# tomershay100/mp3-steganography-lib

Measured on AMD Instinct MI355X. Metric: MP3 frames/sec (decode+re-encode) @44.1kHz stereo 128kbps, 1→8 GPU, higher is better.
Workload: dtype f64 (decode) / int32 (encode); 1 GPU; 10000-frame full decode->stego-embed->re-encode pipeline per MI355X (BASELINE configs[2]); MP3 main data + side info resident in HBM, MP3 frames out; the message cursor chain is decided and the serial chains of the rate loop are checked on the device inside every step; frames_per_gpu=10000, channels=2, message_bits=536, chain_verdict_units_to_redo=0, message_variant_entries=1874, parallelism=frames sharded over 1 GPU(s), no collective

## Files before the change

mp3-steganography-lib_amd/csrc/k_pack.hpp:

```cpp
#pragma once

namespace mp3s {

constexpr int PACK_DW = 372;
constexpr int PACK_FAM = 260;
constexpr int PACK_PT_QUAD = 4 * PACK_FAM, PACK_PT_NONE = PACK_PT_QUAD + 32, PACK_PT = PACK_PT_NONE + 1;
#define MP3S_PS_OVERFLOW 1
#define MP3S_PS_BAD_TABLE 2

__device__ __forceinline__ void lds_put(uint32_t *fb, uint32_t pos, uint32_t val, int n)
{
    if (n <= 0) return;
    const uint32_t d = pos >> 5, o = pos & 31;
    const uint64_t w = (uint64_t)val << (64 - o - n);
    atomicOr(&fb[d], (uint32_t)(w >> 32));
    if ((uint32_t)w) atomicOr(&fb[d + 1], (uint32_t)w);
}

__device__ __forceinline__ int pack_wave_sum(int v, bool on) { return (int)wave_add_u32(on ? (uint32_t)v : 0u); }

__global__ __launch_bounds__(256) void k_enc_pack(
    const int16_t *__restrict__ ix, const mp3s_gr_out *__restrict__ gr, const int32_t *__restrict__ en, int n_frames,
    int sri, int bri, int whole_slots, const uint32_t *__restrict__ frame_off, const uint8_t *__restrict__ padding,
    uint8_t *__restrict__ mp3, int32_t *__restrict__ scfsi_out, int32_t *__restrict__ status, int32_t *__restrict__ sync,
    int f_begin )
{
    __shared__ uint32_t fb3[3][PACK_DW];
    __shared__ uint32_t pt[PACK_PT];
    __shared__ int wg_err;
    const int wave0 = __builtin_amdgcn_readfirstlane(threadIdx.x >> 6), lane0 = threadIdx.x & 63;
    for (int i = threadIdx.x; i < 1024; i += 256) {
        const uint32_t len = i < 256 ? c_tab.hlen13[i] : (i < 512 ? c_tab.hlen15[i - 256] : (i < 768 ? c_tab.hlen16[i - 512] : c_tab.hlen24[i - 768]));
        pt[(i >> 8) * PACK_FAM + (i & 255)] = (&c_tab.hcod[0][0])[i] | (len << 24);
    }
    if (threadIdx.x < 16) {
        pt[PACK_PT_QUAD + threadIdx.x] = (uint32_t)c_tab.hcod_c1a[threadIdx.x] | ((uint32_t)c_tab.hlen_c1a[threadIdx.x] << 24);
        pt[PACK_PT_QUAD + 16 + threadIdx.x] = (15u - threadIdx.x) | (4u << 24);
    }
    if (threadIdx.x == 0) pt[PACK_PT_NONE] = 0;
    for (int i = threadIdx.x; i < 3 * PACK_DW; i += 256) (&fb3[0][0])[i] = 0;
    if (threadIdx.x == 0) wg_err = 0;
    __syncthreads();
    int rot = 0;
    for (int f = f_begin + blockIdx.x; f < n_frames; f += gridDim.x) {
    const int lane = lane0, tid = (int)threadIdx.x;
    int lane_p = lane0, wave = wave0;
    asm volatile("" : "+v"(lane_p), "+s"(wave));
    uint32_t *fb = fb3[rot];
    {
        uint32_t *cl = fb3[rot == 2 ? 0 : rot + 1];
        for (int i = tid; i < PACK_DW; i += 256) cl[i] = 0;
    }
    const int pad = padding[f];
    int p23v[4];
    {
        const int bits_per_frame = 8 * (whole_slots + pad);
        const int mean_bits = (bits_per_frame - 288) / 2;
        int sum = 0;
#pragma unroll
        for (int e = 0; e < 4; e++) {
            p23v[e] = __builtin_amdgcn_readfirstlane(gr[((long)f * 2 + (e & 1)) * 2 + (e >> 1)].part2_3_length);
            sum += p23v[e];
        }
        int stuffing = 2 * mean_bits - sum + ((mean_bits & 1) ? 1 : 0);
        if (stuffing < 0) stuffing = 0;
        if (stuffing) {
            if (p23v[0] + stuffing < 4095) p23v[0] += stuffing;
            else
#pragma unroll
                for (int e = 0; e < 4; e++) {
                    const int extra = 4095 - p23v[e], now = extra < stuffing ? extra : stuffing;
                    p23v[e] += now; stuffing -= now;
                }
        }
    }
    const int e = wave, grn = e >> 1, ch = e & 1;
    const long u = ((long)f * 2 + ch) * 2 + grn;
    const mp3s_gr_out &g = gr[u];
    if (wave < 2) {
        const long u0 = ((long)f * 2 + wave) * 2, u1 = u0 + 1;
        int a = 0, tot21 = 0;
        if (lane_p < 22) {
            a = en[u0 * 22 + lane] - en[u1 * 22 + lane];
            a = a < 0 ? -a : a;
        }
        tot21 = __builtin_amdgcn_readlane(a, 21);
        int sc = lane_p < 21 ? a : 0;
        sc += __builtin_amdgcn_update_dpp(0, sc, 0x111, 0xf, 0xf, false);
        sc += __builtin_amdgcn_update_dpp(0, sc, 0x112, 0xf, 0xf, false);
        sc += __builtin_amdgcn_update_dpp(0, sc, 0x114, 0xf, 0xf, false);
        sc += __builtin_amdgcn_update_dpp(0, sc, 0x118, 0xf, 0xf, false);
        const int row0 = __builtin_amdgcn_readlane(sc, 15);
        const int p5 = __builtin_amdgcn_readlane(sc, 5), p10 = __builtin_amdgcn_readlane(sc, 10), q20 = __builtin_amdgcn_readlane(sc, 20);
        const int tp = row0 + q20;
        int cond = 2 + (gr[u0].xrmax != 0) + (gr[u1].xrmax != 0);
        if (tot21 < 10) cond++;
        if (tp < 100) cond++;
        const int band_sum[4] = {p5, p10 - p5, row0 - p10, q20};
        uint32_t scbits = 0;
#pragma unroll
        for (int b = 0; b < 4; b++) {
            const int s0 = band_sum[b];
            const int v = (cond == 6 && s0 < 10) ? 1 : 0;
            scbits = (scbits << 1) | (uint32_t)v;
            if (lane_p == 0) scfsi_out[((long)f * 2 + wave) * 4 + b] = v;
        }
        if (lane_p == 0) {
            lds_put(fb, 44 + 4 * wave, scbits, 4);
            if (wave == 0) {
                const uint32_t h = (0x7ffu << 21) | (3u << 19) | (1u << 17) | (1u << 16) | ((uint32_t)bri << 12) |
                                   ((uint32_t)(sri % 3) << 10) | ((uint32_t)pad << 9) | (1u << 2);
                fb[0] = h;
            }
        }
    }
    if (lane_p < 4) {
        const uint32_t f0 = ((uint32_t)p23v[e] << 9) | (uint32_t)g.big_values;
        const uint32_t f1 = (((uint32_t)(g.quantizer_step + 210) & 0xff) << 5);
        const uint32_t f2 = ((uint32_t)g.table_select[0] << 10) | ((uint32_t)g.table_select[1] << 5) | (uint32_t)g.table_select[2];
        const uint32_t f3 = ((uint32_t)g.region0_count << 6) | ((uint32_t)g.region1_count << 3) | (uint32_t)g.count1table_select;
        const uint32_t v = lane_p == 0 ? f0 : (lane_p == 1 ? f1 : (lane_p == 2 ? f2 : f3));
        const int n = lane_p == 0 ? 21 : (lane_p == 1 ? 13 : (lane_p == 2 ? 15 : 10));
        const uint32_t at = lane_p == 0 ? 0u : (lane_p == 1 ? 21u : (lane_p == 2 ? 34u : 49u));
        lds_put(fb, 52 + 59 * (uint32_t)e + at, v, n);
    }

    const int ts0 = g.table_select[0], ts1 = g.table_select[1], ts2 = g.table_select[2], c1sel = g.count1table_select;
    uint32_t ustart = 288;
#pragma unroll
    for (int k = 0; k < 3; k++) ustart += k < e ? (uint32_t)p23v[k] : 0u;
    const int bv = g.big_values, c1 = g.count1;
    const int32_t *sfb = c_tab.sfb_long[sri];
    const int r1s = sfb[g.region0_count + 1], r2s = sfb[g.region0_count + 1 + g.region1_count + 1];
    int xv[10];
    {
        const uint32_t *xp = reinterpret_cast<const uint32_t *>(ix + u * 576 + lane * 10);
#pragma unroll
        for (int k = 0; k < 5; k++) {
            const uint32_t w = (lane_p * 5 + k) < 288 ? xp[k] : 0u;
            xv[2 * k] = (int)(int16_t)(w & 0xffff); xv[2 * k + 1] = (int)(int16_t)(w >> 16);
        }
    }
    uint32_t c2[6];
#pragma unroll
    for (int k = 0; k < 5; k++) c2[k] = (uint32_t)((xv[2 * k] & 1) | ((xv[2 * k + 1] & 1) << 1));
    c2[5] = (uint32_t)__builtin_amdgcn_update_dpp(0, (int)c2[0], 0x130, 0xf, 0xf, false);
    uint32_t code0[5], code1[5]; int n0[5], n1[5];
    int tot = 0;
    uint32_t Kr[3];
    bool any_bad = false;
    {
        const int tsr[3] = {ts0, ts1, ts2};
#pragma unroll
        for (int r = 0; r < 3; r++) {
            const int ti = tsr[r];
            const int fam = ti == 13 ? 0 : (ti == 15 ? 1 : (ti < 24 ? 2 : 3));
            Kr[r] = ti ? (uint32_t)fam | ((uint32_t)lin_bits_of(ti) << 2) | (1u << 6) : 0u;
            const int lo = r == 0 ? 0 : (r == 1 ? r1s : r2s), hi = r == 0 ? r1s : (r == 1 ? r2s : 576);
            any_bad |= ti != 0 && ti != 13 && ti != 15 && ti < 16 && lo < 2 * bv && lo < hi;
        }
    }
    const uint32_t quad_base = (uint32_t)(PACK_PT_QUAD + (c1sel ? 16 : 0));
#pragma unroll
    for (int k = 0; k < 5; k++) {
        const int p = lane * 5 + k;
        const int vx = xv[2 * k], vy = xv[2 * k + 1];
        const uint32_t x = (uint32_t)(vx < 0 ? -vx : vx), y = (uint32_t)(vy < 0 ? -vy : vy);
        const int i = 2 * p;
        const uint32_t K = i >= r2s ? Kr[2] : (i >= r1s ? Kr[1] : Kr[0]);
        const uint32_t Ke = p < bv ? K : 0u;
        const bool in_c1 = (uint32_t)(p - bv) < (uint32_t)(2 * c1);
        const uint32_t lb = __builtin_amdgcn_ubfe(Ke, 2, 4);
        const uint32_t lbx = x > 14 ? lb : 0u, lby = y > 14 ? lb : 0u;
        const uint32_t nzx = x < 1 ? x : 1u, nzy = y < 1 ? y : 1u;
        uint32_t ext = __builtin_amdgcn_ubfe(x - 15u, 0, lbx);
        ext = (ext << nzx) | ((uint32_t)vx >> 31);
        ext = (ext << lby) | __builtin_amdgcn_ubfe(y - 15u, 0, lby);
        ext = (ext << nzy) | ((uint32_t)vy >> 31);
        const uint32_t xb = lbx + nzx + lby + nzy;
        const bool inside = Ke != 0 || in_c1;
        const uint32_t xx = x > 14 ? 15u : x, yy = y > 14 ? 15u : y;
        const uint32_t q = (c2[k] | (c2[k + 1] << 2)) & 15u;
        const bool quad = in_c1 && !((p - bv) & 1);
        const uint32_t tix = Ke != 0 ? (Ke & 3u) * (uint32_t)PACK_FAM + xx * 16u + yy : (quad ? quad_base + q : (uint32_t)PACK_PT_NONE);
        const uint32_t word = pt[tix];
        code0[k] = word & 0xffffffu;
        n0[k] = (int)(word >> 24);
        code1[k] = inside ? ext : 0u;
        n1[k] = inside ? (int)xb : 0;
        tot += n0[k] + n1[k];
    }
    const int incl = (int)wave_scan_u32((uint32_t)tot);
    const int huff_bits = __builtin_amdgcn_readlane(incl, 63);
    if (tot) {
        const uint32_t pos0 = ustart + (uint32_t)(incl - tot);
        uint32_t d = pos0 >> 5;
        uint32_t cnt = pos0 & 31u;
        uint64_t top = 0;
        auto append = [&](uint32_t v, int n) {
            top |= (uint64_t)v << ((64u - cnt - (uint32_t)n) & 63u);
            cnt += (uint32_t)n;
            atomicOr(&fb[d], (uint32_t)(top >> 32));
            const uint32_t adv = cnt >> 5;
            top <<= 32u * adv; d += adv; cnt &= 31u;
        };
#pragma unroll
        for (int k = 0; k < 5; k++) { append(code0[k], n0[k]); append(code1[k], n1[k]); }
        atomicOr(&fb[d], (uint32_t)(top >> 32));
    }
    const int p23 = e == 0 ? p23v[0] : (e == 1 ? p23v[1] : (e == 2 ? p23v[2] : p23v[3]));
    if (huff_bits > p23 || any_bad) { if (lane_p == 0) atomicOr(&wg_err, any_bad ? MP3S_PS_BAD_TABLE : MP3S_PS_OVERFLOW); }
    else
        for (uint32_t s = ustart + huff_bits + 32u * lane; s < ustart + (uint32_t)p23; s += 64u * 32u) {
            const uint32_t n = (ustart + p23 - s) < 32u ? (ustart + p23 - s) : 32u;
            lds_put(fb, s, n == 32 ? 0xffffffffu : ((1u << n) - 1), (int)n);
        }
    __syncthreads();
    const int nbytes = whole_slots + pad;
    const uint32_t off = frame_off[f];
    auto byte_at = [&](int k) -> uint32_t { return (fb[k >> 2] >> (24 - 8 * (k & 3))) & 0xffu; };
    const int head = (int)((4u - (off & 3u)) & 3u) < nbytes ? (int)((4u - (off & 3u)) & 3u) : nbytes;
    const int n_dw = (nbytes - head) >> 2, tail0 = head + 4 * n_dw;
    if (tid < head) mp3[off + tid] = (uint8_t)byte_at(tid);
    uint32_t *outw = reinterpret_cast<uint32_t *>(mp3 + off + head);
    {
        const int hq = head >> 2, hs = 8 * (head & 3);
        for (int j = tid; j < n_dw; j += 256) {
            const uint32_t hi = fb[hq + j], lo = fb[hq + j + 1];
            const uint32_t be = hs ? __builtin_amdgcn_alignbit(hi, lo, 32 - hs) : hi;
            outw[j] = __builtin_bswap32(be);
        }
    }
    if (tid < nbytes - tail0) mp3[off + tail0 + tid] = (uint8_t)byte_at(tail0 + tid);
    rot = rot == 2 ? 0 : rot + 1;
    }
    __syncthreads();
    if (threadIdx.x != 0) return;
    const int g = wg_err;
    if (!sync) {
        if (g) atomicOr(status, g);
        return;
    }
    unsigned all;
    if (arrive_with_bits(sync, (unsigned)g, gridDim.x, &all)) *status = (int32_t)all;
}

}
```

Before: 19.65 million frames/s.

## Pre-align frame bitbuffer to output offset, batch Huffman codeword stores, double-buffer LDS

The LDS frame bitbuffer is now written at a bit offset that matches the output byte alignment, so the copy-out becomes aligned dword stores with no alignbit shifting. The same copy-out loop clears each dword as it reads it, which allows two LDS buffers instead of three and drops the separate clear of the next buffer. Each lane's five Huffman codewords are merged into a single up-to-128-bit value and written with at most five stores, using plain stores for words the lane owns alone and atomicOr only at shared edges. The older serial append path remains as a fallback for long codewords. Table-select attributes move into a small LDS lookup table read through readfirstlane.

Result: no change. 19.81 million frames/s, median of 6 (+0.8%).

```diff
diff --git a/mp3-steganography-lib_amd/csrc/k_pack.hpp b/mp3-steganography-lib_amd/csrc/k_pack.hpp
--- a/mp3-steganography-lib_amd/csrc/k_pack.hpp
+++ b/mp3-steganography-lib_amd/csrc/k_pack.hpp
@@ -25,8 +25,9 @@
     uint8_t *__restrict__ mp3, int32_t *__restrict__ scfsi_out, int32_t *__restrict__ status, int32_t *__restrict__ sync,
     int f_begin )
 {
-    __shared__ uint32_t fb3[3][PACK_DW];
+    __shared__ uint32_t fb2[2][PACK_DW];
     __shared__ uint32_t pt[PACK_PT];
+    __shared__ uint32_t kt[32];
     __shared__ int wg_err;
     const int wave0 = __builtin_amdgcn_readfirstlane(threadIdx.x >> 6), lane0 = threadIdx.x & 63;
     for (int i = threadIdx.x; i < 1024; i += 256) {
@@ -38,7 +39,11 @@
         pt[PACK_PT_QUAD + 16 + threadIdx.x] = (15u - threadIdx.x) | (4u << 24);
     }
     if (threadIdx.x == 0) pt[PACK_PT_NONE] = 0;
-    for (int i = threadIdx.x; i < 3 * PACK_DW; i += 256) (&fb3[0][0])[i] = 0;
+    if (threadIdx.x < 32) {
+        const int ti = (int)threadIdx.x;
+        kt[ti] = ti ? (uint32_t)family_of(ti) | ((uint32_t)lin_bits_of(ti) << 2) | (1u << 6) | ((ti != 13 && ti != 15 && ti < 16) ? 1u << 7 : 0u) : 0u;
+    }
+    for (int i = threadIdx.x; i < 2 * PACK_DW; i += 256) (&fb2[0][0])[i] = 0;
     if (threadIdx.x == 0) wg_err = 0;
     __syncthreads();
     int rot = 0;
@@ -46,12 +51,10 @@
     const int lane = lane0, tid = (int)threadIdx.x;
     int lane_p = lane0, wave = wave0;
     asm volatile("" : "+v"(lane_p), "+s"(wave));
-    uint32_t *fb = fb3[rot];
-    {
-        uint32_t *cl = fb3[rot == 2 ? 0 : rot + 1];
-        for (int i = tid; i < PACK_DW; i += 256) cl[i] = 0;
-    }
+    uint32_t *fb = fb2[rot];
     const int pad = padding[f];
+    const uint32_t off = (uint32_t)__builtin_amdgcn_readfirstlane((int)frame_off[f]);
+    const uint32_t a = off & 3u, base = 8u * a;
     int p23v[4];
     {
         const int bits_per_frame = 8 * (whole_slots + pad);
@@ -106,11 +109,11 @@
             if (lane_p == 0) scfsi_out[((long)f * 2 + wave) * 4 + b] = v;
         }
         if (lane_p == 0) {
-            lds_put(fb, 44 + 4 * wave, scbits, 4);
+            lds_put(fb, base + 44 + 4 * wave, scbits, 4);
             if (wave == 0) {
                 const uint32_t h = (0x7ffu << 21) | (3u << 19) | (1u << 17) | (1u << 16) | ((uint32_t)bri << 12) |
                                    ((uint32_t)(sri % 3) << 10) | ((uint32_t)pad << 9) | (1u << 2);
-                fb[0] = h;
+                lds_put(fb, base, h, 32);
             }
         }
     }
@@ -122,11 +125,11 @@
         const uint32_t v = lane_p == 0 ? f0 : (lane_p == 1 ? f1 : (lane_p == 2 ? f2 : f3));
         const int n = lane_p == 0 ? 21 : (lane_p == 1 ? 13 : (lane_p == 2 ? 15 : 10));
         const uint32_t at = lane_p == 0 ? 0u : (lane_p == 1 ? 21u : (lane_p == 2 ? 34u : 49u));
-        lds_put(fb, 52 + 59 * (uint32_t)e + at, v, n);
+        lds_put(fb, base + 52 + 59 * (uint32_t)e + at, v, n);
     }
 
     const int ts0 = g.table_select[0], ts1 = g.table_select[1], ts2 = g.table_select[2], c1sel = g.count1table_select;
-    uint32_t ustart = 288;
+    uint32_t ustart = 288 + base;
 #pragma unroll
     for (int k = 0; k < 3; k++) ustart += k < e ? (uint32_t)p23v[k] : 0u;
     const int bv = g.big_values, c1 = g.count1;
@@ -146,30 +149,29 @@
     for (int k = 0; k < 5; k++) c2[k] = (uint32_t)((xv[2 * k] & 1) | ((xv[2 * k + 1] & 1) << 1));
     c2[5] = (uint32_t)__builtin_amdgcn_update_dpp(0, (int)c2[0], 0x130, 0xf, 0xf, false);
     uint32_t code0[5], code1[5]; int n0[5], n1[5];
-    int tot = 0;
     uint32_t Kr[3];
     bool any_bad = false;
     {
         const int tsr[3] = {ts0, ts1, ts2};
 #pragma unroll
         for (int r = 0; r < 3; r++) {
-            const int ti = tsr[r];
-            const int fam = ti == 13 ? 0 : (ti == 15 ? 1 : (ti < 24 ? 2 : 3));
-            Kr[r] = ti ? (uint32_t)fam | ((uint32_t)lin_bits_of(ti) << 2) | (1u << 6) : 0u;
+            Kr[r] = (uint32_t)__builtin_amdgcn_readfirstlane((int)kt[tsr[r] & 31]);
             const int lo = r == 0 ? 0 : (r == 1 ? r1s : r2s), hi = r == 0 ? r1s : (r == 1 ? r2s : 576);
-            any_bad |= ti != 0 && ti != 13 && ti != 15 && ti < 16 && lo < 2 * bv && lo < hi;
+            any_bad |= (Kr[r] & 128u) != 0 && lo < 2 * bv && lo < hi;
         }
     }
     const uint32_t quad_base = (uint32_t)(PACK_PT_QUAD + (c1sel ? 16 : 0));
+    const int l5 = lane * 5;
+    const int d_r1 = ((r1s + 1) >> 1) - l5, d_r2 = ((r2s + 1) >> 1) - l5, d_bv = bv - l5, d_c1 = d_bv + 2 * c1;
+    uint32_t pw[5]; int pn[5];
+    int nmax = 0;
 #pragma unroll
     for (int k = 0; k < 5; k++) {
-        const int p = lane * 5 + k;
         const int vx = xv[2 * k], vy = xv[2 * k + 1];
         const uint32_t x = (uint32_t)(vx < 0 ? -vx : vx), y = (uint32_t)(vy < 0 ? -vy : vy);
-        const int i = 2 * p;
-        const uint32_t K = i >= r2s ? Kr[2] : (i >= r1s ? Kr[1] : Kr[0]);
-        const uint32_t Ke = p < bv ? K : 0u;
-        const bool in_c1 = (uint32_t)(p - bv) < (uint32_t)(2 * c1);
+        const uint32_t K = k >= d_r2 ? Kr[2] : (k >= d_r1 ? Kr[1] : Kr[0]);
+        const uint32_t Ke = k < d_bv ? K : 0u;
+        const bool in_c1 = k >= d_bv && k < d_c1;
         const uint32_t lb = __builtin_amdgcn_ubfe(Ke, 2, 4);
         const uint32_t lbx = x > 14 ? lb : 0u, lby = y > 14 ? lb : 0u;
         const uint32_t nzx = x < 1 ? x : 1u, nzy = y < 1 ? y : 1u;
@@ -181,19 +183,45 @@
         const bool inside = Ke != 0 || in_c1;
         const uint32_t xx = x > 14 ? 15u : x, yy = y > 14 ? 15u : y;
         const uint32_t q = (c2[k] | (c2[k + 1] << 2)) & 15u;
-        const bool quad = in_c1 && !((p - bv) & 1);
+        const bool quad = in_c1 && !((k - d_bv) & 1);
         const uint32_t tix = Ke != 0 ? (Ke & 3u) * (uint32_t)PACK_FAM + xx * 16u + yy : (quad ? quad_base + q : (uint32_t)PACK_PT_NONE);
         const uint32_t word = pt[tix];
         code0[k] = word & 0xffffffu;
         n0[k] = (int)(word >> 24);
         code1[k] = inside ? ext : 0u;
         n1[k] = inside ? (int)xb : 0;
-        tot += n0[k] + n1[k];
-    }
+        pw[k] = (code0[k] << n1[k]) | code1[k];
+        pn[k] = n0[k] + n1[k];
+        nmax = pn[k] > nmax ? pn[k] : nmax;
+    }
+    const int ncde = pn[2] + pn[3] + pn[4];
+    const int tot = pn[0] + pn[1] + ncde;
     const int incl = (int)wave_scan_u32((uint32_t)tot);
     const int huff_bits = __builtin_amdgcn_readlane(incl, 63);
-    if (tot) {
-        const uint32_t pos0 = ustart + (uint32_t)(incl - tot);
+    const uint32_t end = ustart + (uint32_t)incl, pos0 = end - (uint32_t)tot;
+    if (__builtin_amdgcn_ballot_w64(nmax > 32 || ncde > 63) == 0) {
+        if (tot) {
+            const uint64_t ab = ((uint64_t)pw[0] << pn[1]) | pw[1];
+            const uint64_t cd = ((uint64_t)pw[2] << pn[3]) | pw[3];
+            const uint64_t cde = (cd << pn[4]) | pw[4];
+            const uint32_t r = (uint32_t)ncde & 31u;
+            const bool up = ncde > 31;
+            const uint64_t al = (uint64_t)(uint32_t)ab << r, ah = (uint64_t)(uint32_t)(ab >> 32) << r;
+            const uint32_t a0 = (uint32_t)al, a1 = (uint32_t)(al >> 32) | (uint32_t)ah, a2 = (uint32_t)(ah >> 32);
+            const uint32_t x3 = (uint32_t)cde | (up ? 0u : a0), x2 = (uint32_t)(cde >> 32) | (up ? a0 : a1), x1 = up ? a1 : a2, x0 = up ? a2 : 0u;
+            const uint32_t t = end & 31u, de = end >> 5, span = de - (pos0 >> 5);
+            const uint32_t z0 = __builtin_amdgcn_alignbit(x3, 0u, t), z1 = __builtin_amdgcn_alignbit(x2, x3, t), z2 = __builtin_amdgcn_alignbit(x1, x2, t),
+                           z3 = __builtin_amdgcn_alignbit(x0, x1, t), z4 = x0 >> t;
+            uint32_t *pe = fb + de;
+            if (z0) atomicOr(pe, z0);
+            if (z1) { if (t != 0 && span > 1) pe[-1] = z1; else atomicOr(pe - 1, z1); }
+            if (span > 1) {
+                if (z2) { if (span > 2) pe[-2] = z2; else atomicOr(pe - 2, z2); }
+                if (z3) { if (span > 3) pe[-3] = z3; else atomicOr(pe - 3, z3); }
+                if (z4) atomicOr(pe - 4, z4);
+            }
+        }
+    } else if (tot) {
         uint32_t d = pos0 >> 5;
         uint32_t cnt = pos0 & 31u;
         uint64_t top = 0;
@@ -216,23 +244,21 @@
             lds_put(fb, s, n == 32 ? 0xffffffffu : ((1u << n) - 1), (int)n);
         }
     __syncthreads();
-    const int nbytes = whole_slots + pad;
-    const uint32_t off = frame_off[f];
-    auto byte_at = [&](int k) -> uint32_t { return (fb[k >> 2] >> (24 - 8 * (k & 3))) & 0xffu; };
-    const int head = (int)((4u - (off & 3u)) & 3u) < nbytes ? (int)((4u - (off & 3u)) & 3u) : nbytes;
-    const int n_dw = (nbytes - head) >> 2, tail0 = head + 4 * n_dw;
-    if (tid < head) mp3[off + tid] = (uint8_t)byte_at(tid);
-    uint32_t *outw = reinterpret_cast<uint32_t *>(mp3 + off + head);
-    {
-        const int hq = head >> 2, hs = 8 * (head & 3);
-        for (int j = tid; j < n_dw; j += 256) {
-            const uint32_t hi = fb[hq + j], lo = fb[hq + j + 1];
-            const uint32_t be = hs ? __builtin_amdgcn_alignbit(hi, lo, 32 - hs) : hi;
-            outw[j] = __builtin_bswap32(be);
-        }
-    }
-    if (tid < nbytes - tail0) mp3[off + tail0 + tid] = (uint8_t)byte_at(tail0 + tid);
-    rot = rot == 2 ? 0 : rot + 1;
+    {
+        const int first = (int)a, last = first + whole_slots + pad;
+        uint8_t *out = mp3 + (off - a);
+        for (int k = tid; k < PACK_DW; k += 256) {
+            const uint32_t v = fb[k];
+            fb[k] = 0;
+            const int b0 = 4 * k;
+            if (b0 >= first && b0 + 4 <= last) reinterpret_cast<uint32_t *>(out)[k] = __builtin_bswap32(v);
+            else
+#pragma unroll
+                for (int b = 0; b < 4; b++)
+                    if (b0 + b >= first && b0 + b < last) out[b0 + b] = (uint8_t)(v >> (24 - 8 * b));
+        }
+    }
+    rot ^= 1;
     }
     __syncthreads();
     if (threadIdx.x != 0) return;
```
